# lcrekko/lq_mpc

Hardware: AMD Instinct MI355X
Metric: MPC QP-steps/sec (batched systems) at n_x=4,n_u=2,N=10; 1/2/4/8 GPU (higher is better)
Workload: dtype f64

## Files before the change

### lq_mpc_amd/csrc/lqmpc_r16.hip

```cpp
#include <cstdio>
#include "lqmpc_r16_body.h"
#include "lqmpc_launch.h"

namespace lqmpc {

template <int NX, int NU, int N, int MODE, int LPI>
__global__ void __launch_bounds__(64, (R16Build<NX, NU, N, LPI>::WAVES)) lqmpc_r16_kernel(KParams p)
{
    using C = R16<NX, NU, N, LPI, (R16Build<NX, NU, N, LPI>::OCC == 2)>;
    __shared__ double lds_raw[C::IPW * C::INST];
    r16_body<NX, NU, N, MODE, LPI, R16Build<NX, NU, N, LPI>::OCC>(p, lds_raw, (long long)blockIdx.x * C::IPW, p.Bsz);
}

template <int NX, int NU, int N, int LPI>
static void launch_r16_one(const KParams &p, hipStream_t stream)
{
    constexpr int IPW = 64 / LPI;
    const dim3 grid((unsigned)((p.Bsz + IPW - 1) / IPW));
    if (p.mode == MODE_SOLVE) hipLaunchKernelGGL((lqmpc_r16_kernel<NX, NU, N, MODE_SOLVE, LPI>), grid, dim3(64), 0, stream, p);
    else if (p.mode == MODE_MAXVN) hipLaunchKernelGGL((lqmpc_r16_kernel<NX, NU, N, MODE_MAXVN, LPI>), grid, dim3(64), 0, stream, p);
    else if (p.mode == MODE_SWEEP) hipLaunchKernelGGL((lqmpc_r16_kernel<NX, NU, N, MODE_SWEEP, LPI>), grid, dim3(64), 0, stream, p);
    else {
#ifdef LQMPC_R16_PROF
        long long z[32] = {0};
        (void)hipMemcpyToSymbol(HIP_SYMBOL(g_r16_prof), z, sizeof z);
#endif
        hipLaunchKernelGGL((lqmpc_r16_kernel<NX, NU, N, MODE_ROLLOUT, LPI>), grid, dim3(64), 0, stream, p);
#ifdef LQMPC_R16_PROF
        (void)hipStreamSynchronize(stream);
        (void)hipMemcpyFromSymbol(z, HIP_SYMBOL(g_r16_prof), sizeof z);
        fprintf(stderr, "r16 prof (block %d ticks): set-up on the matrix core %lld v_r %lld | rollout %lld\n", PROFBLK, z[5], z[6], z[7]);
        fprintf(stderr, "r16 prof (grid): waves %lld  set-up %.0f  total %.0f ticks/wave | free wave-steps %lld at %.0f ticks | busy wave-steps %lld at %.0f ticks, "
                "%.2f wave-iterations each (steps 1..T-1); %lld wave-iterations on the general (primal-capable) path in all\n", z[15], (double)z[13] / z[15], (double)z[14] / z[15], z[10], (double)z[8] / (z[10] ? z[10] : 1),
                z[11], (double)z[9] / (z[11] ? z[11] : 1), (double)z[12] / (z[11] ? z[11] : 1), z[16]);
        fprintf(stderr, "r16 prof (grid, ticks/wave): set-up on the matrix core %.0f v_r %.0f\n", (double)z[22] / z[15], (double)z[23] / z[15]);
        fprintf(stderr, "r16 prof (grid): %lld dual-only wave-iterations at %.0f ticks, %lld general at %.0f ticks\n", z[26], (double)z[24] / (z[26] ? z[26] : 1), z[16],
                (double)z[25] / (z[16] ? z[16] : 1));
        fprintf(stderr, "r16 prof (grid): step 0: %.0f ticks/wave, %.2f wave-iterations/wave, %.2f of them general; %lld of %lld wavefronts ever took the general (P-reading) path\n",
                (double)z[27] / z[15], (double)z[28] / z[15], (double)z[29] / z[15], z[30], z[15]);
#endif
    }
}

#define R16E(NX, NU, N) {NX, NU, N, 16, "lqmpc_r16_kernel<" #NX "," #NU "," #N ">", launch_r16_one<NX, NU, N, 16>}
#define R64E(NX, NU, N) {NX, NU, N, 64, "lqmpc_r64_kernel<" #NX "," #NU "," #N ">", launch_r16_one<NX, NU, N, 64>}
static const ShapeEntry g_r16[] = {
    R16E(4, 2, 10),
    R16E(2, 1, 10),
    R16E(2, 1, 5), R16E(2, 1, 6), R16E(2, 1, 7), R16E(2, 1, 8), R16E(2, 1, 9),
    R16E(2, 1, 20), R16E(2, 1, 30),
    R64E(4, 2, 20),
};

static const ShapeEntry *find_r16(int nx, int nu, int N)
{
    for (const ShapeEntry &e : g_r16)
        if (e.nx == nx && e.nu == nu && e.N == N) return &e;
    return nullptr;
}

bool r16_available(int nx, int nu, int N) { return find_r16(nx, nu, N) != nullptr; }
int r16_lanes(int nx, int nu, int N) { const ShapeEntry *e = find_r16(nx, nu, N); return e ? e->lpi : 0; }

bool launch_r16(const KParams &p, hipStream_t stream, const char **name)
{
    const ShapeEntry *e = find_r16(p.nx, p.nu, p.N);
    if (!e) return false;
    const bool lat = e->lpi == 16 && (p.r16_build >= 0 ? p.r16_build == 1 : p.Bsz <= 4096);
    if (!(lat && launch_r16_lat(p, stream))) e->launch(p, stream);
    if (name) *name = e->name;
    return true;
}

}
```

### lq_mpc_amd/csrc/lqmpc_r16_body.h

```cpp
#pragma once
#include "lqmpc_wg_linalg.h"
#include "lqmpc_r16_setup.h"

namespace lqmpc {

using wg::ldsd;
using wg::ldsi;
using wg::rowb;
using wg::fmac_rowb;
using wg::fmac_rowb_self;
using wg::fmac_rowb4;
using wg::fmac_rowb_self4;
using wg::fmac_rowb_self2;
using wg::fmac_rowb_self3;
using wg::fmac_rowb_lanes4;
using wg::fmac_rowb_lanes4x2;
using wg::dpp_settle;

#ifdef LQMPC_R16_PROF
__device__ long long g_r16_prof[32];
#define RPROF(k) do { const long long now_ = clock64(); if (threadIdx.x == 0 && blockIdx.x == PROFBLK) g_r16_prof[k] += now_ - prof_t; if (k < 7) prof_ph[k] += now_ - prof_t; prof_t = clock64(); } while (0)
#define RPROF_START long long prof_t = clock64()
#define RPROF_ADD(k, v) do { if (threadIdx.x == 0) atomicAdd((unsigned long long *)&g_r16_prof[k], (unsigned long long)(v)); } while (0)
#ifndef PROFBLK
#define PROFBLK 0
#endif
#else
#define RPROF(k) do { } while (0)
#define RPROF_START do { } while (0)
#define RPROF_ADD(k, v) do { } while (0)
#endif

typedef unsigned long long mask_t;

template <int NX, int NU, int N, int LPI = 16, bool PACKED = false>
struct R16 {
    static constexpr int n = N * NU;
    static constexpr int RB = (n + LPI - 1) / LPI;
    static constexpr int IPW = 64 / LPI;
    static constexpr int CS = 4 * (((n + 1) / 2 + 3) / 4);
    static constexpr int LDW = n + 1;
    static constexpr int PK = PACKED ? n * (n + 1) / 2 : n * LDW;
    static constexpr int VEC = LPI * RB;
    static constexpr int oP = 0, oW = PK, oR = 2 * PK, oX = oR + VEC, oY = oX + VEC, oL = oY + VEC;
    static constexpr int oC = oL + CS / 2;
    static constexpr int CN0 = 3 * NX * NX + NU * NU + NX * NU;
    static constexpr int CN1 = (NX > NU ? NX : NU) * (2 * NX + 2 * NU);
    static constexpr int CN = CN0 > CN1 ? CN0 : CN1;
    static constexpr int oG = (NX > 8) ? oR : 0;
    static constexpr int SETUP = oG + n * NX;
    static constexpr int END = oC + CN + (CN & 1);
    static constexpr int oD = (END > SETUP) ? END : SETUP;
    static constexpr int INST = oD + 2;
    static constexpr int MAXIT = 12;
    static_assert(LPI == 16 || LPI == 64, "a DPP row or the whole wavefront");
    static_assert((n + 1) / 2 <= CS && n <= 64, "the smaller side must fit the gathered system");
};

template <int NX, int NU, int N, int LPI>
struct R16Build {
    static constexpr int OCC = ((LPI == 16 && N * NU > 10) || LPI == 64 || NX > 8) ? 2 : 1;
    static constexpr long long LDS_BYTES = (long long)(64 / LPI) * R16<NX, NU, N, LPI, (OCC == 2)>::INST * 8;
    static constexpr int WAVES = ((OCC == 2 || (N * NU <= 10 && LPI == 16)) && LDS_BYTES * 8 <= 160 * 1024) ? 2 : 1;
};

template <int LPI>
__device__ __forceinline__ mask_t iballot(bool c, int q)
{
    if constexpr (LPI == 16) return (__ballot(c) >> (16 * q)) & 0xFFFFull;
    else return __ballot(c);
}
template <int LPI>
__device__ __forceinline__ double ibcast(double x, int k)
{
    if constexpr (LPI == 16) return rowb(x, k);
    else return wg::rdlane(x, k);
}
template <int LPI>
__device__ __forceinline__ void ifmac_self4(double *acc, double y, int k)
{
    if constexpr (LPI == 16) fmac_rowb_self4(acc[0], acc[1], acc[2], acc[3], y, k);
    else {
#pragma unroll
        for (int e = 0; e < 4; ++e) acc[e] = __builtin_fma(wg::rdlane(acc[e], k), y, acc[e]);
    }
}
template <int LPI, int K, int CS>
__device__ __forceinline__ void ifmac_self_tail(double (&S)[CS], double &rhs, double g)
{
    constexpr int r = K % 4;
    if constexpr (LPI == 16) {
        if constexpr (r == 0) fmac_rowb_self4(S[K + 1], S[K + 2], S[K + 3], rhs, g, K);
        else if constexpr (r == 1) fmac_rowb_self3(S[K + 1], S[K + 2], rhs, g, K);
        else if constexpr (r == 2) fmac_rowb_self2(S[K + 1], rhs, g, K);
        else fmac_rowb_self(rhs, g, K);
    } else {
#pragma unroll
        for (int j = K + 1; j < 4 * (K / 4) + 4; ++j) S[j] = __builtin_fma(wg::rdlane(S[j], K), g, S[j]);
        rhs = __builtin_fma(wg::rdlane(rhs, K), g, rhs);
    }
}
template <int LPI>
__device__ __forceinline__ void isettle(double &x)
{
    if constexpr (LPI == 16) dpp_settle(x);
}
__device__ __forceinline__ int rowb_i(int x, int c)
{
    switch (c) {
#define LQMPC_X(C) case C: return __builtin_amdgcn_update_dpp(0, x, 0x150 + C, 0xF, 0xF, true);
        LQMPC_ROWB_CASES(LQMPC_X)
#undef LQMPC_X
    }
    return x;
}
__device__ __forceinline__ unsigned row_or(unsigned x)
{
    x |= (unsigned)__builtin_amdgcn_update_dpp(0, (int)x, 0x128, 0xF, 0xF, false);
    x |= (unsigned)__builtin_amdgcn_update_dpp(0, (int)x, 0x124, 0xF, 0xF, false);
    x |= (unsigned)__builtin_amdgcn_update_dpp(0, (int)x, 0x122, 0xF, 0xF, false);
    x |= (unsigned)__builtin_amdgcn_update_dpp(0, (int)x, 0x121, 0xF, 0xF, false);
    return x;
}
__device__ __forceinline__ unsigned row_umax(unsigned x)
{
    x = max(x, (unsigned)__builtin_amdgcn_update_dpp(0, (int)x, 0x128, 0xF, 0xF, false));
    x = max(x, (unsigned)__builtin_amdgcn_update_dpp(0, (int)x, 0x124, 0xF, 0xF, false));
    x = max(x, (unsigned)__builtin_amdgcn_update_dpp(0, (int)x, 0x122, 0xF, 0xF, false));
    x = max(x, (unsigned)__builtin_amdgcn_update_dpp(0, (int)x, 0x121, 0xF, 0xF, false));
    return x;
}

template <int NX, int NU, int N, int MODE, int LPI = 16, int OCC = 1>
__device__ __forceinline__ void r16_body(const KParams &p, double *lds_raw, long long slot0, long long slot_end)
{
    constexpr bool PACKED = (OCC == 2);
    using C = R16<NX, NU, N, LPI, PACKED>;
    constexpr int CS = C::CS;
    constexpr int n = C::n, RB = C::RB, LDW = C::LDW;
    constexpr int REC = NX * NX + NX * NU + NX;
    const int lane = threadIdx.x, q = lane / LPI, i = lane % LPI;
    ldsd *L = (ldsd *)lds_raw + q * C::INST;
    ldsd *Pp = L + C::oP, *Wp = L + C::oW, *rL = L + C::oR, *xL = L + C::oX, *yL = L + C::oY;
    ldsi *list = (ldsi *)(L + C::oL);
    const long long Bsz = p.Bsz;
    const long long b_raw = slot0 + q;
    const bool valid = b_raw < slot_end;
    const long long slot = valid ? b_raw : slot_end - 1;
    const long long b = p.perm ? (long long)p.perm[slot] : slot;
    const double *sh = p.sh;
    const mask_t nmask = (n == 64) ? ~0ull : ((1ull << n) - 1ull);

    int rw[RB], tri[RB];
    bool vrow[RB];
#pragma unroll
    for (int s = 0; s < RB; ++s) {
        rw[s] = i + LPI * s;
        tri[s] = rw[s] * (rw[s] + 1) / 2;
        vrow[s] = rw[s] < n;
    }

    auto ad = [&](int r, int tr, int j) -> int { if constexpr (PACKED) return (j <= r) ? tr + j : j * (j + 1) / 2 + r; else return r * LDW + j; };
    auto ad2 = [&](int a, int b2) -> int {
        if constexpr (PACKED) { const int hi = a > b2 ? a : b2, lo = a > b2 ? b2 : a; return hi * (hi + 1) / 2 + lo; }
        else return a * LDW + b2;
    };

    double G[RB][NX], vr[RB];
    constexpr bool CTL_F = MODE == MODE_CTL_FACTOR, CTL_S = MODE == MODE_CTL_STEP, CTL_R = MODE == MODE_CTL_ROLL;
    constexpr bool CTL_REC = CTL_S || CTL_R;
    using CR = CtlRecT<NX, NU, N>;
    constexpr bool LAZY_P = (LPI == 64 && !CTL_F) || CTL_REC;
    bool P_ready = !LAZY_P;
    bool W_ready = !CTL_REC;
    bool face_stays = false;
    auto tri_rc = [](int e, int &r, int &c) {
        r = (int)((__builtin_sqrtf(8.0f * (float)e + 1.0f) - 1.0f) * 0.5f);
        r = ((r + 1) * (r + 2) / 2 <= e) ? r + 1 : r;
        r = (r * (r + 1) / 2 > e) ? r - 1 : r;
        c = e - r * (r + 1) / 2;
    };
#ifdef LQMPC_NO_ROLL
    constexpr bool ROLL = false;
#else
    constexpr bool ROLL = LPI == 16 && NX <= 8 && N * ((NX + 3) / 4) <= 12 && MODE != MODE_MAXVN && !CTL_F && !CTL_REC;
#endif
    unsigned cold32[2] = {0u, 0u};
    bool cold_armed = false;
#ifdef LQMPC_R16_PROF
    const long long prof_t0 = clock64();
    int prof_wit = 0, prof_slow = 0, prof_fast = 0;
    long long prof_slowt = 0;
    long long prof_ph[8] = {0, 0, 0, 0, 0, 0, 0, 0};
#endif
    if constexpr (CTL_REC) {
        const double *rc = p.ctl_rec + b * p.ctl_stride;
#pragma unroll
        for (int s = 0; s < RB; ++s) {
            const int mr = vrow[s] ? rw[s] : 0;
#pragma unroll
            for (int a = 0; a < NX; ++a) G[s][a] = rc[CR::oG + mr * NX + a];
            vr[s] = vrow[s] ? rc[CR::oV + mr] : 0.0;
        }
    } else {
        RPROF_START;
        long long bg = b;
        ldsd *Lg = L;
        if constexpr (LPI == 16) {
            const int gq = (lane >> 2) & 3;
            const long long sraw = slot0 + gq, sl = sraw < slot_end ? sraw : slot_end - 1;
            bg = p.perm ? (long long)p.perm[sl] : sl;
            Lg = (ldsd *)lds_raw + gq * C::INST;
        }
        if constexpr (NX > 8) {
            static_assert(LPI == 16 && C::oG >= 2 * C::PK, "wide states: four instances per wavefront, G handed over behind P and W");
            r16_setup_wide<NX, NU, N, PACKED, RB>(setup_args(p), bg, Lg, C::oW, C::oG, C::oD);
#pragma unroll
            for (int s = 0; s < RB; ++s) {
#pragma unroll
                for (int a = 0; a < NX; ++a) {
                    const double x = L[C::oG + (vrow[s] ? rw[s] * NX + a : 0)];
                    G[s][a] = vrow[s] ? x : 0.0;
                }
            }
            __syncthreads();
        } else r16_setup_mfma<NX, NU, N, LPI, PACKED, RB, ROLL>(setup_args(p), bg, Lg, L, C::oW, C::oG, C::oD, G, roll_args(p), cold32[0], cold32[1]);
        if constexpr (!LAZY_P) r16_build_P<NX, NU, N, LPI, PACKED>(setup_args(p), bg, Lg, C::oP, C::oD);
        RPROF(5);
        const bool has_lin = p.has_lin != 0;
#pragma unroll
        for (int s = 0; s < RB; ++s) vr[s] = 0.0;
        if (has_lin) {
            if (p.has_ref) {
                double qr[RB];
#pragma unroll
                for (int s = 0; s < RB; ++s) qr[s] = 0.0;
                constexpr bool WIDE = NX > 8;
                double lam[NX], A2[WIDE ? 1 : NX][WIDE ? 1 : NX], B2[WIDE ? 1 : NX][WIDE ? 1 : NU];
                if constexpr (WIDE) {
                    const int ia = i < NX ? i : 0;
                    double Ac[NX], Bc[RB][NX];
#pragma unroll
                    for (int c = 0; c < NX; ++c) {
                        lam[c] = 0.0;
                        Ac[c] = p.rec ? p.rec[b * REC + c * NX + ia] : p.A[(long long)(c * NX + ia) * Bsz + b];
#pragma unroll
                        for (int s = 0; s < RB; ++s)
                            Bc[s][c] = p.rec ? p.rec[b * REC + NX * NX + c * NU + rw[s] % NU] : p.B[(long long)(c * NU + rw[s] % NU) * Bsz + b];
                    }
#pragma unroll 1
                    for (int r = N - 1; r >= 0; --r) {
                        const int oQ = (r < N - 1) ? p.so.Q : p.so.P;
                        double t = 0.0;
#pragma unroll
                        for (int c = 0; c < NX; ++c) t = __builtin_fma(sh[oQ + ia * NX + c], -sh[p.so.xref + c * N + r], t);
#pragma unroll
                        for (int c = 0; c < NX; ++c) t = __builtin_fma(Ac[c], lam[c], t);
                        yL[i] = t;
                        __syncthreads();
#pragma unroll
                        for (int a = 0; a < NX; ++a) lam[a] = yL[a];
                        __syncthreads();
#pragma unroll
                        for (int s = 0; s < RB; ++s) {
                            const int ui = rw[s] % NU;
                            double tk = 0.0;
#pragma unroll
                            for (int a = 0; a < NX; ++a) tk = __builtin_fma(Bc[s][a], lam[a], tk);
#pragma unroll
                            for (int j = 0; j < NU; ++j) tk = __builtin_fma(-sh[p.so.R + ui * NU + j], sh[p.so.uref + j * N + r], tk);
                            qr[s] = (vrow[s] && rw[s] / NU == r) ? 2.0 * tk : qr[s];
                        }
                    }
                } else {
#pragma unroll
                    for (int a = 0; a < NX; ++a) {
                        lam[a] = 0.0;
#pragma unroll
                        for (int c = 0; c < NX; ++c) A2[a][c] = p.rec ? p.rec[b * REC + a * NX + c] : p.A[(long long)(a * NX + c) * Bsz + b];
#pragma unroll
                        for (int k = 0; k < NU; ++k) B2[a][k] = p.rec ? p.rec[b * REC + NX * NX + a * NU + k] : p.B[(long long)(a * NU + k) * Bsz + b];
                    }
#pragma unroll 1
                    for (int r = N - 1; r >= 0; --r) {
                        const int oQ = (r < N - 1) ? p.so.Q : p.so.P;
                        double l2[NX];
#pragma unroll
                        for (int a = 0; a < NX; ++a) {
                            double t = 0.0;
#pragma unroll
                            for (int c = 0; c < NX; ++c) t = __builtin_fma(sh[oQ + a * NX + c], -sh[p.so.xref + c * N + r], t);
#pragma unroll
                            for (int c = 0; c < NX; ++c) t = __builtin_fma(A2[c][a], lam[c], t);
                            l2[a] = t;
                        }
#pragma unroll
                        for (int a = 0; a < NX; ++a) lam[a] = l2[a];
#pragma unroll
                        for (int s = 0; s < RB; ++s) {
                            const int ui = rw[s] % NU;
                            double t = 0.0;
#pragma unroll
                            for (int k = 0; k < NU; ++k) {
                                double tk = 0.0;
#pragma unroll
                                for (int a = 0; a < NX; ++a) tk = __builtin_fma(B2[a][k], lam[a], tk);
#pragma unroll
                                for (int j = 0; j < NU; ++j) tk = __builtin_fma(-sh[p.so.R + k * NU + j], sh[p.so.uref + j * N + r], tk);
                                t = (ui == k) ? tk : t;
                            }
                            qr[s] = (vrow[s] && rw[s] / NU == r) ? 2.0 * t : qr[s];
                        }
                    }
                }
#pragma unroll
                for (int s = 0; s < RB; ++s) xL[rw[s]] = qr[s];
                __syncthreads();
#pragma unroll
                for (int s = 0; s < RB; ++s) {
                    double t = 0.0;
                    const int mr = vrow[s] ? rw[s] : 0, mt = vrow[s] ? tri[s] : 0;
#pragma unroll
                    for (int j = 0; j < n; ++j) t = __builtin_fma(Wp[ad(mr, mt, j)], xL[j], t);
                    vr[s] = -t;
                }
                __syncthreads();
            }
#pragma unroll
            for (int s = 0; s < RB; ++s) {
                const int k = rw[s] % NU;
                vr[s] = vrow[s] ? vr[s] - 0.5 * (sh[p.so.ub + k] + sh[p.so.lb + k]) : 0.0;
            }
        }
        if constexpr (LAZY_P && MODE != MODE_MAXVN) {
            mask_t out = 0;
#pragma unroll
            for (int s = 0; s < RB; ++s) {
                double acc = vr[s];
#pragma unroll
                for (int a = 0; a < NX; ++a) acc = __builtin_fma(G[s][a], p.rec ? p.rec[b * REC + NX * NX + NX * NU + a] : p.x0[(long long)a * Bsz + b], acc);
                const int k = rw[s] % NU;
                out |= iballot<LPI>(vrow[s] && !(fabs(acc) <= 0.5 * (sh[p.so.ub + k] - sh[p.so.lb + k])), q) << (LPI * s);
            }
            if (__ballot(2 * __popcll(out) > n) != 0ull) {
                r16_build_P<NX, NU, N, LPI, PACKED>(setup_args(p), bg, Lg, C::oP, C::oD);
                P_ready = true;
            }
        }
        RPROF(6);
    }
    if constexpr (CTL_F) {
        __syncthreads();
        const long long ir = p.ctl_idx ? (long long)p.ctl_idx[b] : b;
        if (valid && (unsigned long long)ir < (unsigned long long)p.ctl_n) {
            double *rc = p.ctl_rec + ir * p.ctl_stride;
            for (int e = i; e < NX * NX; e += LPI) rc[CR::oA + e] = p.A[(long long)e * Bsz + b];
            for (int e = i; e < NX * NU; e += LPI) rc[CR::oB + e] = p.B[(long long)e * Bsz + b];
#pragma unroll
            for (int s = 0; s < RB; ++s) {
                if (vrow[s]) {
#pragma unroll
                    for (int a = 0; a < NX; ++a) rc[CR::oG + rw[s] * NX + a] = G[s][a];
                    rc[CR::oV + rw[s]] = vr[s];
                }
            }
            for (int e = i; e < CR::tri; e += LPI) {
                int r, c;
                tri_rc(e, r, c);
                rc[CR::oW + e] = Wp[ad2(r, c)];
                rc[CR::oP + e] = Pp[ad2(r, c)];
            }
        }
        return;
    }
    auto ctl_fill = [&](ldsd *M, int off, bool on) {
        const double *src = p.ctl_rec + b * p.ctl_stride + off;
        constexpr int CNT = (CR::tri + LPI - 1) / LPI;
        double val[CNT];
#pragma unroll
        for (int k = 0; k < CNT; ++k) { const int e = i + LPI * k; val[k] = (on && e < CR::tri) ? src[e] : 0.0; }
#pragma unroll
        for (int k = 0; k < CNT; ++k) {
            const int e = i + LPI * k;
            if (on && e < CR::tri) {
                if constexpr (PACKED) M[e] = val[k];
                else { int r, c; tri_rc(e, r, c); M[r * LDW + c] = val[k]; M[c * LDW + r] = val[k]; }
            }
        }
        __syncthreads();
    };
    RPROF_START;
    RPROF_ADD(13, clock64() - prof_t0);

    long long bq = b;
    asm volatile("" : "+v"(bq));
    double h[RB], ctr[RB];
#pragma unroll
    for (int s = 0; s < RB; ++s) {
        const int k = rw[s] % NU;
        h[s] = vrow[s] ? 0.5 * (sh[p.so.ub + k] - sh[p.so.lb + k]) : 1.0;
        ctr[s] = vrow[s] ? 0.5 * (sh[p.so.ub + k] + sh[p.so.lb + k]) : 0.0;
    }
    double Qm[NX][NX], Rm[NU][NU];
    ldsd *cQ = L + C::oC, *cR = cQ + NX * NX;
    if constexpr (MODE == MODE_ROLLOUT || CTL_R) {
    } else if constexpr (OCC == 2) {
        if constexpr (NX > 8) {
            for (int e = i; e < NX * NX; e += LPI) cQ[e] = sh[p.so.Q + e];
            for (int e = i; e < NU * NU; e += LPI) cR[e] = sh[p.so.R + e];
        } else if (i == 0) {
#pragma unroll
            for (int a = 0; a < NX; ++a) {
#pragma unroll
                for (int c = 0; c < NX; ++c) {
                    cQ[a * NX + c] = sh[p.so.Q + a * NX + c];
                }
            }
#pragma unroll
            for (int k = 0; k < NU; ++k)
#pragma unroll
                for (int j = 0; j < NU; ++j) cR[k * NU + j] = sh[p.so.R + k * NU + j];
        }
        __syncthreads();
    } else {
#pragma unroll
        for (int a = 0; a < NX; ++a) {
#pragma unroll
            for (int c = 0; c < NX; ++c) Qm[a][c] = sh[p.so.Q + a * NX + c];
        }
#pragma unroll
        for (int k = 0; k < NU; ++k)
#pragma unroll
            for (int j = 0; j < NU; ++j) Rm[k][j] = sh[p.so.R + k * NU + j];
    }
    auto Qv = [&](int a, int c) -> double { if constexpr (OCC == 2) return cQ[a * NX + c]; else return Qm[a][c]; };
    auto Rv = [&](int k, int j) -> double { if constexpr (OCC == 2) return cR[k * NU + j]; else return Rm[k][j]; };
// ... 505 lines not shown
                        const mask_t bit = 1ull << rw[s];
                        const bool act = vrow[s] && (mA & bit);
                        const bool lo = act ? ((mL & bit) && gl[s] >= -tol) : (vrow[s] && v[s] < -h[s] * (1.0 + 1e-12));
                        const bool up = act ? ((mU & bit) && gl[s] <= tol) : (vrow[s] && v[s] > h[s] * (1.0 + 1e-12));
                        nL |= iballot<LPI>(lo, q) << (LPI * s);
                        nU |= iballot<LPI>(up, q) << (LPI * s);
                        nf = nf || (vrow[s] && !(fabs(v[s]) < 1e300));
                    }
                    const bool rownf = iballot<LPI>(nf, q) != 0;
#ifdef LQMPC_R16_PROF
                    prof_wit += 1; prof_slow += 1; prof_slowt += clock64() - prof_it0;
#endif
                    if (busy) {
                        iters += 1;
                        if (rowfail || rownf) { failed = true; busy = false; }
                        else if (nL == mL && nU == mU) busy = false;
                        else { mL = nL; mU = nU; }
                    }
                    __syncthreads();
                    if (__ballot(busy) == 0ull) break;
                }
            }
        }
        } while (LAZY_P && need_P);
        if (busy) failed = true;
        if (failed || rowbad) {
            status = 3; pL = 0; pU = 0;
#pragma unroll
            for (int s = 0; s < RB; ++s) v[s] = fmin(fmax(vu[s], -h[s]), h[s]);
        } else {
            pL = mL; pU = mU;
        }
    };
    auto stage_input = [&](const double (&v)[RB], int st, double (&u)[NU]) {
#pragma unroll
        for (int k = 0; k < NU; ++k) {
            const int row = st * NU + k;
            const double uk = fmin(fmax(v[row / LPI], -h[row / LPI]), h[row / LPI]) + ctr[row / LPI];
            u[k] = ibcast<LPI>(uk, row % LPI);
        }
    };
    if (MODE != MODE_ROLLOUT && !CTL_R) {
        double Am[NX][NX], Bmm[NX][NU], Pm[NX][NX];
        ldsd *cA = cR + NU * NU, *cB = cA + NX * NX, *cP = cB + NX * NU;
        if constexpr (OCC == 2) {
            if constexpr (NX > 8) {
                for (int e = i; e < NX * NX; e += LPI) {
                    cA[e] = p.rec ? p.rec[bq * REC + e] : p.A[(long long)e * Bsz + bq];
                    cP[e] = sh[p.so.P + e];
                }
                for (int e = i; e < NX * NU; e += LPI) cB[e] = p.rec ? p.rec[bq * REC + NX * NX + e] : p.B[(long long)e * Bsz + bq];
            } else if (i == 0) {
#pragma unroll
                for (int a = 0; a < NX; ++a) {
#pragma unroll
                    for (int c = 0; c < NX; ++c) {
                        if constexpr (CTL_S) cA[a * NX + c] = p.ctl_rec[bq * p.ctl_stride + CR::oA + a * NX + c];
                        else cA[a * NX + c] = p.rec ? p.rec[bq * REC + a * NX + c] : p.A[(long long)(a * NX + c) * Bsz + bq];
                        cP[a * NX + c] = sh[p.so.P + a * NX + c];
                    }
#pragma unroll
                    for (int k = 0; k < NU; ++k) {
                        if constexpr (CTL_S) cB[a * NU + k] = p.ctl_rec[bq * p.ctl_stride + CR::oB + a * NU + k];
                        else cB[a * NU + k] = p.rec ? p.rec[bq * REC + NX * NX + a * NU + k] : p.B[(long long)(a * NU + k) * Bsz + bq];
                    }
                }
            }
            __syncthreads();
        } else {
#pragma unroll
            for (int a = 0; a < NX; ++a) {
#pragma unroll
                for (int c = 0; c < NX; ++c) {
                    if constexpr (CTL_S) Am[a][c] = p.ctl_rec[bq * p.ctl_stride + CR::oA + a * NX + c];
                    else Am[a][c] = p.rec ? p.rec[bq * REC + a * NX + c] : p.A[(long long)(a * NX + c) * Bsz + bq];
                    Pm[a][c] = sh[p.so.P + a * NX + c];
                }
#pragma unroll
                for (int k = 0; k < NU; ++k) {
                    if constexpr (CTL_S) Bmm[a][k] = p.ctl_rec[bq * p.ctl_stride + CR::oB + a * NU + k];
                    else Bmm[a][k] = p.rec ? p.rec[bq * REC + NX * NX + a * NU + k] : p.B[(long long)(a * NU + k) * Bsz + bq];
                }
            }
        }
        auto Av = [&](int a, int c) -> double { if constexpr (OCC == 2) return cA[a * NX + c]; else return Am[a][c]; };
        auto Bv = [&](int a, int k) -> double { if constexpr (OCC == 2) return cB[a * NU + k]; else return Bmm[a][k]; };
        auto Pv = [&](int a, int c) -> double { if constexpr (OCC == 2) return cP[a * NX + c]; else return Pm[a][c]; };
        auto value_fn = [&](const double (&x0v)[NX], const double (&v)[RB]) -> double {
            if constexpr (NX > 8) {
                static_assert(OCC == 2 && LPI == 16, "wide states: constants in LDS, four instances per wavefront");
                const int ia = i < NX ? i : 0, ik = i < NU ? i : 0;
                double xs[NX], cx, cu = 0.0;
#pragma unroll
                for (int a = 0; a < NX; ++a) xs[a] = x0v[a];
                {
                    double xm = xs[0], qx = 0.0;
#pragma unroll
                    for (int a = 1; a < NX; ++a) xm = (i == a) ? xs[a] : xm;
#pragma unroll
                    for (int cc = 0; cc < NX; ++cc) qx = __builtin_fma(cQ[ia * NX + cc], xs[cc], qx);
                    cx = xm * qx;
                }
#pragma unroll
                for (int s = 0; s < RB; ++s) xL[rw[s]] = vrow[s] ? fmin(fmax(v[s], -h[s]), h[s]) + ctr[s] : 0.0;
                __syncthreads();
                int zc = 0;
#pragma unroll 1
                for (int st = 0; st < N; ++st) {
                    asm volatile("" : "+v"(zc));
                    const ldsd *rA = cA + ia * NX + zc, *rB = cB + ia * NU + zc, *rW = ((st == N - 1) ? cP : cQ) + ia * NX + zc, *rR = cR + ik * NU + zc;
                    double u[NU], xm = 0.0, qx = 0.0, ru = 0.0;
#pragma unroll
                    for (int k = 0; k < NU; ++k) u[k] = xL[st * NU + k];
#pragma unroll
                    for (int cc = 0; cc < NX; ++cc) xm = __builtin_fma(rA[cc], xs[cc], xm);
#pragma unroll
                    for (int k = 0; k < NU; ++k) xm = __builtin_fma(rB[k], u[k], xm);
#pragma unroll
                    for (int a = 0; a < NX; ++a) xs[a] = ibcast<LPI>(xm, a);
                    double dm = xm;
                    if (p.has_ref) dm -= sh[p.so.xref + ia * N + st];
#pragma unroll
                    for (int cc = 0; cc < NX; ++cc) qx = __builtin_fma(rW[cc], p.has_ref ? xs[cc] - sh[p.so.xref + cc * N + st] : xs[cc], qx);
                    cx = __builtin_fma(dm, qx, cx);
                    if (p.has_ref) {
#pragma unroll
                        for (int k = 0; k < NU; ++k) u[k] -= sh[p.so.uref + k * N + st];
                    }
                    double um = u[0];
#pragma unroll
                    for (int k = 1; k < NU; ++k) um = (i == k) ? u[k] : um;
#pragma unroll
                    for (int j = 0; j < NU; ++j) ru = __builtin_fma(rR[j], u[j], ru);
                    cu = __builtin_fma(um, ru, cu);
                }
                __syncthreads();
                double c = 0.0;
#pragma unroll
                for (int a = 0; a < NX; ++a) c += ibcast<LPI>(cx, a);
#pragma unroll
                for (int k = 0; k < NU; ++k) c += ibcast<LPI>(cu, k);
                return c;
            }
            double xs[NX], c = 0.0;
#pragma unroll
            for (int a = 0; a < NX; ++a) xs[a] = x0v[a];
#pragma unroll
            for (int a = 0; a < NX; ++a)
#pragma unroll
                for (int cc = 0; cc < NX; ++cc) c = __builtin_fma(xs[a] * Qv(a, cc), xs[cc], c);
#pragma unroll
            for (int s = 0; s < RB; ++s) xL[rw[s]] = vrow[s] ? fmin(fmax(v[s], -h[s]), h[s]) + ctr[s] : 0.0;
            __syncthreads();
#pragma unroll 1
            for (int st = 0; st < N; ++st) {
                double u[NU], xn[NX];
#pragma unroll
                for (int k = 0; k < NU; ++k) u[k] = xL[st * NU + k];
#pragma unroll
                for (int a = 0; a < NX; ++a) {
                    double acc = 0.0;
#pragma unroll
                    for (int cc = 0; cc < NX; ++cc) acc = __builtin_fma(Av(a, cc), xs[cc], acc);
#pragma unroll
                    for (int k = 0; k < NU; ++k) acc = __builtin_fma(Bv(a, k), u[k], acc);
                    xn[a] = acc;
                }
#pragma unroll
                for (int a = 0; a < NX; ++a) { xs[a] = xn[a]; if (p.has_ref) xn[a] -= sh[p.so.xref + a * N + st]; }
#pragma unroll
                for (int a = 0; a < NX; ++a)
#pragma unroll
                    for (int cc = 0; cc < NX; ++cc) c = __builtin_fma(xn[a] * ((st == N - 1) ? Pv(a, cc) : Qv(a, cc)), xn[cc], c);
                if (p.has_ref) {
#pragma unroll
                    for (int k = 0; k < NU; ++k) u[k] -= sh[p.so.uref + k * N + st];
                }
#pragma unroll
                for (int k = 0; k < NU; ++k)
#pragma unroll
                    for (int j = 0; j < NU; ++j) c = __builtin_fma(u[k] * Rv(k, j), u[j], c);
            }
            __syncthreads();
            return c;
        };
        if constexpr (CTL_S) {
            double x[NX], v[RB], u[NU];
#pragma unroll
            for (int a = 0; a < NX; ++a) x[a] = p.x0[(long long)a * Bsz + bq];
            unsigned long long *fc = p.ctl_face + bq * (2 + 2 * NX);
            pL = fc[0]; pU = fc[1];
            {
                double dprev = 0.0, dnext = 0.0;
#pragma unroll
                for (int a = 0; a < NX; ++a) {
                    const double e0 = x[a] - __longlong_as_double((long long)fc[2 + a]);
                    const double e1 = x[a] - __longlong_as_double((long long)fc[2 + NX + a]);
                    dprev = __builtin_fma(e0, e0, dprev);
                    dnext = __builtin_fma(e1, e1, dnext);
                }
                face_stays = dprev < dnext;
            }
            qp(x, v);
            double vn = 0.0;
            if (p.VN) vn = value_fn(x, v);
            stage_input(v, 0, u);
            if (writer) {
                fc[0] = pL; fc[1] = pU;
#pragma unroll
                for (int a = 0; a < NX; ++a) {
                    double xn = 0.0;
#pragma unroll
                    for (int cc = 0; cc < NX; ++cc) xn = __builtin_fma(Av(a, cc), x[cc], xn);
#pragma unroll
                    for (int k = 0; k < NU; ++k) xn = __builtin_fma(Bv(a, k), u[k], xn);
                    fc[2 + a] = (unsigned long long)__double_as_longlong(x[a]);
                    fc[2 + NX + a] = (unsigned long long)__double_as_longlong(xn);
                }
                if (p.VN) p.VN[b] = vn;
#pragma unroll
                for (int k = 0; k < NU; ++k) p.u0[(long long)k * Bsz + bq] = u[k];
            }
        } else if (MODE == MODE_SOLVE) {
            double x[NX], v[RB], u[NU];
#pragma unroll
            for (int a = 0; a < NX; ++a) x[a] = p.rec ? p.rec[bq * REC + NX * NX + NX * NU + a] : p.x0[(long long)a * Bsz + bq];
            cold_armed = ROLL;
            qp(x, v);
            const double vn = value_fn(x, v);
            stage_input(v, 0, u);
            if (writer) {
                p.VN[b] = vn;
#pragma unroll
                for (int k = 0; k < NU; ++k) p.u0[(long long)k * Bsz + bq] = u[k];
            }
        } else {
            double best = -1e308;
            for (int kk = 0; kk < p.K; ++kk) {
                double x[NX], v[RB];
#pragma unroll
                for (int a = 0; a < NX; ++a) x[a] = sh[p.so.x0s + a * p.K + kk];
                pL = 0; pU = 0;
                qp(x, v);
                const double vn = value_fn(x, v);
                best = (vn > best || vn != vn) ? vn : best;
            }
            if (writer) p.MV[b] = best;
        }
    }
    if (MODE == MODE_ROLLOUT || MODE == MODE_SWEEP || CTL_R) {
        pL = 0; pU = 0;
        double x[NX];
#pragma unroll
        for (int a = 0; a < NX; ++a) {
            if constexpr (CTL_R) x[a] = p.x0[(long long)a * Bsz + bq];
            else x[a] = p.rec ? p.rec[bq * REC + NX * NX + NX * NU + a] : p.x0[(long long)a * Bsz + bq];
        }
        int ia = i < NX ? i : 0, ik = i < NU ? i : 0;
        asm volatile("" : "+v"(ia), "+v"(ik));
        double Qr_[NX], Ar_[NX], Br_[NU], Rr_[NU];
#pragma unroll
        for (int c = 0; c < NX; ++c) {
            Qr_[c] = sh[p.so.Q + ia * NX + c];
            Ar_[c] = p.true_per_instance ? p.At[(long long)(ia * NX + c) * Bsz + bq] : sh[p.so.At + ia * NX + c];
        }
#pragma unroll
        for (int k = 0; k < NU; ++k) {
            Br_[k] = p.true_per_instance ? p.Bt[(long long)(ia * NU + k) * Bsz + bq] : sh[p.so.Bt + ia * NU + k];
            Rr_[k] = sh[p.so.R + ik * NU + k];
        }
        constexpr bool ROWS_IN_LDS = OCC == 2 && LPI == 64 && 2 * NX + 2 * NU > 12;
        constexpr int RW = 2 * NX + 2 * NU;
        static_assert((NX > NU ? NX : NU) * RW <= C::CN + (C::CN & 1), "the per-lane rows fit the constants region");
        ldsd *myc = L + C::oC + ((i < NX || i < NU) ? i : 0) * RW;
        if constexpr (ROWS_IN_LDS) {
            __syncthreads();
            if (i < NX || i < NU) {
#pragma unroll
                for (int c = 0; c < NX; ++c) { myc[c] = Ar_[c]; myc[NX + NU + c] = Qr_[c]; }
#pragma unroll
                for (int k = 0; k < NU; ++k) { myc[NX + k] = Br_[k]; myc[2 * NX + NU + k] = Rr_[k]; }
            }
            __syncthreads();
        }
        auto Ar = [&](int c) -> double { if constexpr (ROWS_IN_LDS) return myc[c]; else return Ar_[c]; };
        auto Br = [&](int k) -> double { if constexpr (ROWS_IN_LDS) return myc[NX + k]; else return Br_[k]; };
        auto Qr = [&](int c) -> double { if constexpr (ROWS_IN_LDS) return myc[NX + NU + c]; else return Qr_[c]; };
        auto Rr = [&](int k) -> double { if constexpr (ROWS_IN_LDS) return myc[2 * NX + NU + k]; else return Rr_[k]; };
        double costx, costu = 0.0;
        {
            double xm = x[0], qx = 0.0;
#pragma unroll
            for (int a = 1; a < NX; ++a) xm = (i == a) ? x[a] : xm;
#pragma unroll
            for (int c = 0; c < NX; ++c) qx = __builtin_fma(Qr(c), x[c], qx);
            costx = xm * qx;
        }
        if (p.X && writer) {
#pragma unroll
            for (int a = 0; a < NX; ++a) p.X[((long long)a * (p.T + 1)) * Bsz + bq] = x[a];
        }
#ifdef LQMPC_R16_PROF
        long long prof_ts = 0, prof_acc[5] = {0, 0, 0, 0, 0};
#endif
        for (int t = 0; t < p.T; ++t) {
            double v[RB], u[NU], xn[NX];
#ifdef LQMPC_R16_PROF
            if (t == 1) { RPROF_ADD(27, clock64() - prof_ts); RPROF_ADD(28, prof_wit); RPROF_ADD(29, prof_slow); }
            if (t > 0) {
                const long long d_ = clock64() - prof_ts;
                if (prof_wit) { prof_acc[1] += d_; prof_acc[3] += 1; prof_acc[4] += prof_wit; } else { prof_acc[0] += d_; prof_acc[2] += 1; }
            }
            prof_ts = clock64();
            prof_wit = 0;
#endif
            bool inside = false;
            {
                bool out = false;
#pragma unroll
                for (int s = 0; s < RB; ++s) {
                    double acc = vr[s];
#pragma unroll
                    for (int a = 0; a < NX; ++a) acc = __builtin_fma(G[s][a], x[a], acc);
                    v[s] = acc;
                    out = out || (vrow[s] && !(fabs(acc) <= h[s]));
                }
                inside = __ballot(out) == 0ull;
            }
            cold_armed = ROLL && t == 0;
            if (inside) { pL = 0; pU = 0; }
            else qp(x, v);
            const double um = fmin(fmax(v[0], -h[0]), h[0]) + ctr[0];
            stage_input(v, 0, u);
            double xm = 0.0, qx = 0.0, ru = 0.0;
#pragma unroll
            for (int c = 0; c < NX; ++c) xm = __builtin_fma(Ar(c), x[c], xm);
#pragma unroll
            for (int k = 0; k < NU; ++k) xm = __builtin_fma(Br(k), u[k], xm);
#pragma unroll
            for (int a = 0; a < NX; ++a) xn[a] = ibcast<LPI>(xm, a);
#pragma unroll
            for (int a = 0; a < NX; ++a) x[a] = xn[a];
#pragma unroll
            for (int c = 0; c < NX; ++c) qx = __builtin_fma(Qr(c), xn[c], qx);
            costx = __builtin_fma(xm, qx, costx);
#pragma unroll
            for (int j = 0; j < NU; ++j) ru = __builtin_fma(Rr(j), u[j], ru);
            costu = __builtin_fma(um, ru, costu);
            if (writer) {
                if (p.X) {
#pragma unroll
                    for (int a = 0; a < NX; ++a) p.X[((long long)a * (p.T + 1) + t + 1) * Bsz + bq] = xn[a];
                }
                if (p.U) {
#pragma unroll
                    for (int k = 0; k < NU; ++k) p.U[((long long)k * p.T + t) * Bsz + bq] = u[k];
                }
            }
        }
        double cost = 0.0;
#pragma unroll
        for (int a = 0; a < NX; ++a) cost += ibcast<LPI>(costx, a);
#pragma unroll
        for (int k = 0; k < NU; ++k) cost += ibcast<LPI>(costu, k);
        RPROF(7);
#ifdef LQMPC_R16_PROF
        for (int k_ = 0; k_ < 5; ++k_) RPROF_ADD(8 + k_, prof_acc[k_]);
#endif
        RPROF_ADD(14, clock64() - prof_t0); RPROF_ADD(15, 1); RPROF_ADD(16, prof_slow); RPROF_ADD(30, prof_slow > 0 ? 1 : 0);
#ifdef LQMPC_R16_PROF
        for (int k_ = 0; k_ < 8; ++k_) RPROF_ADD(17 + k_, prof_ph[k_]);
        RPROF_ADD(25, prof_slowt); RPROF_ADD(26, prof_fast);
#endif
        if (writer) p.JT[b] = cost;
    }
    if (writer) {
        if (p.status) p.status[b] = status;
        if (p.iters) p.iters[b] = iters;
        if (status == 3 && p.fail_list) p.fail_list[atomicAdd(p.fail_count, 1)] = (int)b;
    }
}

}
```

Before: 7.376 billion.

## Speculatively roll out chunks of unconstrained MPC steps with one deferred check

In rollout mode for the two benchmark shapes, once a step is found inside the unconstrained region, the kernel speculatively advances up to eight steps using only the unclamped affine control law. It accumulates an out-of-bounds ballot across the chunk and commits it if no row was active, otherwise it restores the saved state and cost and falls back to per-step processing until a QP runs again. This removes the per-step ballot branch and the clamping and stage_input overhead on long free stretches. The risk is wasted work when a chunk gets discarded, plus extra register pressure from the saved state.

```diff
diff --git a/lq_mpc_amd/csrc/lqmpc_r16.hip b/lq_mpc_amd/csrc/lqmpc_r16.hip
--- a/lq_mpc_amd/csrc/lqmpc_r16.hip
+++ b/lq_mpc_amd/csrc/lqmpc_r16.hip
@@ -9,7 +9,7 @@
 {
     using C = R16<NX, NU, N, LPI, (R16Build<NX, NU, N, LPI>::OCC == 2)>;
     __shared__ double lds_raw[C::IPW * C::INST];
-    r16_body<NX, NU, N, MODE, LPI, R16Build<NX, NU, N, LPI>::OCC>(p, lds_raw, (long long)blockIdx.x * C::IPW, p.Bsz);
+    r16_body<NX, NU, N, MODE, LPI, R16Build<NX, NU, N, LPI>::OCC, (MODE == MODE_ROLLOUT && R16Build<NX, NU, N, LPI>::CHUNKS)>(p, lds_raw, (long long)blockIdx.x * C::IPW, p.Bsz);
 }
 
 template <int NX, int NU, int N, int LPI>
@@ -22,7 +22,7 @@
     else if (p.mode == MODE_SWEEP) hipLaunchKernelGGL((lqmpc_r16_kernel<NX, NU, N, MODE_SWEEP, LPI>), grid, dim3(64), 0, stream, p);
     else {
 #ifdef LQMPC_R16_PROF
-        long long z[32] = {0};
+        long long z[36] = {0};
         (void)hipMemcpyToSymbol(HIP_SYMBOL(g_r16_prof), z, sizeof z);
 #endif
         hipLaunchKernelGGL((lqmpc_r16_kernel<NX, NU, N, MODE_ROLLOUT, LPI>), grid, dim3(64), 0, stream, p);
@@ -38,6 +38,8 @@
                 (double)z[25] / (z[16] ? z[16] : 1));
         fprintf(stderr, "r16 prof (grid): step 0: %.0f ticks/wave, %.2f wave-iterations/wave, %.2f of them general; %lld of %lld wavefronts ever took the general (P-reading) path\n",
                 (double)z[27] / z[15], (double)z[28] / z[15], (double)z[29] / z[15], z[30], z[15]);
+        fprintf(stderr, "r16 prof (grid): chunks of iteration-free steps: %lld committed, %lld discarded with %lld steps computed for nothing (%.2f %% of the free wave-steps)\n",
+                z[31], z[32], z[33], 100.0 * (double)z[33] / (z[10] ? z[10] : 1));
 #endif
     }
 }
diff --git a/lq_mpc_amd/csrc/lqmpc_r16_body.h b/lq_mpc_amd/csrc/lqmpc_r16_body.h
--- a/lq_mpc_amd/csrc/lqmpc_r16_body.h
+++ b/lq_mpc_amd/csrc/lqmpc_r16_body.h
@@ -18,7 +18,7 @@
 using wg::dpp_settle;
 
 #ifdef LQMPC_R16_PROF
-__device__ long long g_r16_prof[32];
+__device__ long long g_r16_prof[36];
 #define RPROF(k) do { const long long now_ = clock64(); if (threadIdx.x == 0 && blockIdx.x == PROFBLK) g_r16_prof[k] += now_ - prof_t; if (k < 7) prof_ph[k] += now_ - prof_t; prof_t = clock64(); } while (0)
 #define RPROF_START long long prof_t = clock64()
 #define RPROF_ADD(k, v) do { if (threadIdx.x == 0) atomicAdd((unsigned long long *)&g_r16_prof[k], (unsigned long long)(v)); } while (0)
@@ -62,6 +62,7 @@
     static constexpr int OCC = ((LPI == 16 && N * NU > 10) || LPI == 64 || NX > 8) ? 2 : 1;
     static constexpr long long LDS_BYTES = (long long)(64 / LPI) * R16<NX, NU, N, LPI, (OCC == 2)>::INST * 8;
     static constexpr int WAVES = ((OCC == 2 || (N * NU <= 10 && LPI == 16)) && LDS_BYTES * 8 <= 160 * 1024) ? 2 : 1;
+    static constexpr bool CHUNKS = NX == 4 && NU == 2 && ((LPI == 16 && N == 10) || (LPI == 64 && N == 20));
 };
 
 template <int LPI>
@@ -131,7 +132,7 @@
     return x;
 }
 
-template <int NX, int NU, int N, int MODE, int LPI = 16, int OCC = 1>
+template <int NX, int NU, int N, int MODE, int LPI = 16, int OCC = 1, bool CHUNKS = false>
 __device__ __forceinline__ void r16_body(const KParams &p, double *lds_raw, long long slot0, long long slot_end)
 {
     constexpr bool PACKED = (OCC == 2);
@@ -1243,18 +1244,74 @@
         }
 #ifdef LQMPC_R16_PROF
         long long prof_ts = 0, prof_acc[5] = {0, 0, 0, 0, 0};
+        int prof_nst = 1;
 #endif
+        constexpr int FREE_KMAX = 8;
+        const bool free_chunks = CHUNKS && !p.X && !p.U;
+        bool prev_free = false, chunk_hold = false;
+        mask_t rows_mask[RB];
+#pragma unroll
+        for (int s = 0; s < RB; ++s) rows_mask[s] = __ballot(vrow[s]);
         for (int t = 0; t < p.T; ++t) {
             double v[RB], u[NU], xn[NX];
 #ifdef LQMPC_R16_PROF
             if (t == 1) { RPROF_ADD(27, clock64() - prof_ts); RPROF_ADD(28, prof_wit); RPROF_ADD(29, prof_slow); }
             if (t > 0) {
                 const long long d_ = clock64() - prof_ts;
-                if (prof_wit) { prof_acc[1] += d_; prof_acc[3] += 1; prof_acc[4] += prof_wit; } else { prof_acc[0] += d_; prof_acc[2] += 1; }
+                if (prof_wit) { prof_acc[1] += d_; prof_acc[3] += 1; prof_acc[4] += prof_wit; } else { prof_acc[0] += d_; prof_acc[2] += prof_nst; }
             }
             prof_ts = clock64();
             prof_wit = 0;
+            prof_nst = 1;
 #endif
+            if (free_chunks && prev_free && !chunk_hold && p.T - t >= 2) {
+                const int kc = p.T - t < FREE_KMAX ? p.T - t : FREE_KMAX;
+                double x_keep[NX];
+                const double costx_keep = costx, costu_keep = costu;
+#pragma unroll
+                for (int a = 0; a < NX; ++a) x_keep[a] = x[a];
+                mask_t outside = 0;
+#pragma unroll 1
+                for (int j = 0; j < kc; ++j) {
+#pragma unroll
+                    for (int s = 0; s < RB; ++s) {
+                        double acc = vr[s];
+#pragma unroll
+                        for (int a = 0; a < NX; ++a) acc = __builtin_fma(G[s][a], x[a], acc);
+                        v[s] = acc;
+                        outside |= __ballot(!(fabs(acc) <= h[s])) & rows_mask[s];
+                    }
+                    const double um = v[0] + ctr[0];
+#pragma unroll
+                    for (int k = 0; k < NU; ++k) u[k] = ibcast<LPI>(um, k);
+                    double xm = 0.0, qx = 0.0, ru = 0.0;
+#pragma unroll
+                    for (int c = 0; c < NX; ++c) xm = __builtin_fma(Ar(c), x[c], xm);
+#pragma unroll
+                    for (int k = 0; k < NU; ++k) xm = __builtin_fma(Br(k), u[k], xm);
+#pragma unroll
+                    for (int a = 0; a < NX; ++a) x[a] = ibcast<LPI>(xm, a);
+#pragma unroll
+                    for (int c = 0; c < NX; ++c) qx = __builtin_fma(Qr(c), x[c], qx);
+                    costx = __builtin_fma(xm, qx, costx);
+#pragma unroll
+                    for (int j2 = 0; j2 < NU; ++j2) ru = __builtin_fma(Rr(j2), u[j2], ru);
+                    costu = __builtin_fma(um, ru, costu);
+                }
+                if (outside == 0ull) {
+#ifdef LQMPC_R16_PROF
+                    prof_nst = kc;
+                    RPROF_ADD(31, 1);
+#endif
+                    t += kc - 1;
+                    continue;
+                }
+                RPROF_ADD(32, 1); RPROF_ADD(33, kc);
+#pragma unroll
+                for (int a = 0; a < NX; ++a) x[a] = x_keep[a];
+                costx = costx_keep; costu = costu_keep;
+                chunk_hold = true;
+            }
             bool inside = false;
             {
                 bool out = false;
@@ -1270,7 +1327,8 @@
             }
             cold_armed = ROLL && t == 0;
             if (inside) { pL = 0; pU = 0; }
-            else qp(x, v);
+            else { qp(x, v); chunk_hold = false; }
+            prev_free = inside;
             const double um = fmin(fmax(v[0], -h[0]), h[0]) + ctr[0];
             stage_input(v, 0, u);
             double xm = 0.0, qx = 0.0, ru = 0.0;
```

After: 7.717 billion (median of 6 runs). 1.05x the previous value.
